# wenlinlee/FISCO-BCOS

Measured on AMD Instinct MI355X. Metric: sigs_per_sec, higher is better.
Workload: dtype u32 (256-bit integer); 1 GPU; C2; txs_total=10000, txs_rank0=10000, parallelism=dp1 (tx-index shards)

## Files before the change

fisco-bcos_amd/csrc/ecc_coop.hip:

```cpp
#include "ecc_device.h"
#include "ec26_trio.h"

namespace bcosgpu {

struct SplitLds {
    uint32_t tab[8][16][64];
    uint32_t zc[8][64];
    uint32_t u1[8][64];
    uint32_t k1[4][64];
    uint32_t k2[4][64];
    uint32_t flags[64];
    uint32_t pt[3][25][64];
};

__device__ __forceinline__ void lds_store_jac(uint32_t (*dst)[64], const Jac& P, int lane) {
    lds_store_fe(dst, P.X, lane);
    lds_store_fe(dst + 8, P.Y, lane);
    lds_store_fe(dst + 16, P.Z, lane);
    dst[24][lane] = P.inf ? 1u : 0u;
}
__device__ __forceinline__ void lds_load_jac(Jac& P, const uint32_t (*src)[64], int lane) {
    lds_load_fe(P.X, src, lane);
    lds_load_fe(P.Y, src + 8, lane);
    lds_load_fe(P.Z, src + 16, lane);
// ... 831 lines not shown
    for (int i = 0; i < lo; ++i) shr_bits<BITS>(k);
    CurveK1x::set_inf(acc);
    uint32_t b = k.v[0] & MASK;
    shr_bits<BITS>(k);
    const uint4* e = reinterpret_cast<const uint4*>(tab + (static_cast<size_t>(lo) * E + b) * 16);
    uint4 q0 = e[0], q1 = e[1], q2 = e[2], q3 = e[3];
#pragma unroll 1
    for (int i = lo; i < hi; ++i) {
        const uint32_t bi = b;
        Aff26 T;
        {
            const uint32_t x[8] = {q0.x, q0.y, q0.z, q0.w, q1.x, q1.y, q1.z, q1.w};
            const uint32_t y[8] = {q2.x, q2.y, q2.z, q2.w, q3.x, q3.y, q3.z, q3.w};
            fe26_from_words(T.x, x);
            fe26_from_words(T.y, y);
        }
        const int in = i + 1 < hi ? i + 1 : i;
        b = k.v[0] & MASK;
        shr_bits<BITS>(k);
        e = reinterpret_cast<const uint4*>(tab + (static_cast<size_t>(in) * E + b) * 16);
        q0 = e[0];
        q1 = e[1];
        q2 = e[2];
        q3 = e[3];
        Jac26 S;
        CurveK1x::madd(S, acc, T);
        CurveK1x::cmov(acc, S, bi != 0u);
    }
}

__device__ __forceinline__ void coop26_store_jac(uint32_t (*dst)[64], const Jac26& P, int lane) {
    fe X, Y, Z;
    fe26_to_fe(X, P.X);
    fe26_to_fe(Y, P.Y);
    fe26_to_fe(Z, P.Z);
    Jac J;
    fe_copy(J.X, X);
    fe_copy(J.Y, Y);
    fe_copy(J.Z, Z);
    J.inf = P.inf;
    coop_store_jac(dst, J, lane);
}
__device__ __forceinline__ void coop26_load_jac(Jac26& P, const uint32_t (*src)[64], int lane) {
    Jac J;
    coop_load_jac(J, src, lane);
    fe26_from_fe(P.X, J.X);
    fe26_from_fe(P.Y, J.Y);
    fe26_from_fe(P.Z, J.Z);
    P.inf = J.inf;
}
__device__ __forceinline__ void lds_load_fe26(fe26& a, const uint32_t (*src)[64], int lane) {
    fe w;
    lds_load_fe(w, src, lane);
    fe26_from_fe(a, w);
}
__device__ __forceinline__ void lds_store_fe26(uint32_t (*dst)[64], const fe26& a, int lane) {
    fe w;
    fe26_to_fe(w, a);
    lds_store_fe(dst, w, lane);
}

constexpr int kTrioWords = 31;
struct Trio26Lds {
    uint32_t tab[8][20][64];
    uint32_t tabphx[8][10][64];
    uint32_t zc[8][64];
    uint32_t k[2][4][64];
    uint32_t flags[64];
    uint32_t pt[5][25][64];
    uint32_t xe[8][64];
    uint32_t xrinv[8][64];
    uint32_t ys[8][64];
    uint32_t rflag[64];
    uint32_t post[3];
};
struct Trio26RecoverLds : Trio26Lds {
    uint32_t sq[10][40];
    uint32_t yok[64];
    uint32_t spost[kTfSlots];
    uint32_t hpost[4];
    uint32_t xg[2][kTrioWords][64];
    uint32_t tsuf[6][10][64];
    uint32_t kw[10][64];
};
__device__ __forceinline__ void lds_flag_wait4(uint32_t* a, uint32_t* b, uint32_t* c, uint32_t* d) {
    for (;;) {
        const uint32_t x = __hip_atomic_load(a, __ATOMIC_RELAXED, __HIP_MEMORY_SCOPE_WORKGROUP);
        const uint32_t y = __hip_atomic_load(b, __ATOMIC_RELAXED, __HIP_MEMORY_SCOPE_WORKGROUP);
        const uint32_t z = __hip_atomic_load(c, __ATOMIC_RELAXED, __HIP_MEMORY_SCOPE_WORKGROUP);
        const uint32_t u = __hip_atomic_load(d, __ATOMIC_RELAXED, __HIP_MEMORY_SCOPE_WORKGROUP);
        if (x != 0u && y != 0u && z != 0u && u != 0u) break;
        __builtin_amdgcn_s_sleep(1);
    }
    __builtin_amdgcn_fence(__ATOMIC_ACQUIRE, "workgroup");
}
struct TrioTableFlags {
    uint32_t* f;
    __device__ __forceinline__ void post(int s) { lds_flag_post(f + s); }
    __device__ __forceinline__ void wait(int s) { lds_flag_wait(f + s); }
    __device__ __forceinline__ void stamp(int k) {
        COOP_T(k);
        (void)k;
    }
};
__device__ __forceinline__ void lds_store_limbs26(uint32_t (*dst)[64], const fe26& a, int lane) {
    fe26 t;
    fe26_copy(t, a);
    fe26_normalize(t);
#pragma unroll
    for (int q = 0; q < 10; ++q) dst[q][lane] = t.v[q];
}

__device__ __forceinline__ void trio_store(uint32_t* buf, const TrioPt& P, int lane) {
#pragma unroll
    for (int q = 0; q < 10; ++q) {
        buf[q * 64 + lane] = P.S1.v[q];
        buf[(10 + q) * 64 + lane] = P.Xs.v[q];
        buf[(20 + q) * 64 + lane] = P.Zs.v[q];
    }
    buf[30 * 64 + lane] = P.inf ? 1u : 0u;
}
__device__ __forceinline__ void trio_load(TrioPt& P, const uint32_t* buf, int lane) {
#pragma unroll
    for (int q = 0; q < 10; ++q) {
        P.S1.v[q] = buf[q * 64 + lane];
        P.Xs.v[q] = buf[(10 + q) * 64 + lane];
        P.Zs.v[q] = buf[(20 + q) * 64 + lane];
    }
    P.inf = buf[30 * 64 + lane] != 0u;
}
__device__ __forceinline__ void trio_from_jac(TrioPt& P, const Jac26& J, const TrioLane& T) {
    trio::sel(P.S1, T.r0, J.X, J.Y);
    fe26_copy(P.Xs, J.X);
    fe26_copy(P.Zs, J.Z);
    P.inf = J.inf;
}

__device__ __forceinline__ void trio_entry(Aff26& S, const Trio26Lds& L, int tl, int d, bool neg, bool phi) {
    const uint32_t m = static_cast<uint32_t>((d < 0 ? -d : d) - 1) & 7u;
    const uint32_t* base = &L.tab[0][0][0] + m * (20 * 64) + tl;
    const uint32_t* bx = phi ? &L.tabphx[0][0][0] + m * (10 * 64) + tl : base;
#pragma unroll
    for (int q = 0; q < 10; ++q) {
        S.x.v[q] = bx[q * 64];
        S.y.v[q] = base[(10 + q) * 64];
    }
    F26_SETM(S.x, 1);
    F26_SETM(S.y, 1);
    fe26 ny;
    fe26_neg<2>(ny, S.y);
    fe26_cmov(S.y, ny, (d < 0) != neg);
}

__device__ __forceinline__ void trio_glv_chain(TrioPt& acc, const Trio26Lds& L, int chain, int tl, uint32_t tflags,
                                               const TrioLane& T) {
    fe k;
    fe_zero(k);
#pragma unroll
    for (int q = 0; q < 4; ++q) k.v[q] = L.k[chain][q][tl];
    const bool neg = chain == 0 ? (tflags & 4u) != 0 : (tflags & 8u) != 0;
    const bool phi = chain == 1;
    trio_chain_start(acc, k.v[3], [&](Aff26& S, int d) { trio_entry(S, L, tl, d, neg, phi); }, T);
    shl4_128(k);
    TrioAcc la;
    trio_acc_from(la, acc);
#pragma unroll 1
    for (int w = 30; w >= 0; --w)
        trio_window(la, booth_digit128(k), [&](Aff26& S, int d) { trio_entry(S, L, tl, d, neg, phi); }, T);
    trio_acc_to(acc, la, T);
}

template <bool WITH0, bool WITH2>
__device__ __forceinline__ void trio_sum_partials(TrioPt& A, const Trio26Lds& L, int tl, const TrioLane& T) {
    Jac26 Ga, Gb;
    TrioPt B;
    coop26_load_jac(Ga, L.pt[3], tl);
    coop26_load_jac(Gb, L.pt[4], tl);
    trio_from_jac(A, Ga, T);
    trio_from_jac(B, Gb, T);
    trio_add(A, A, B, T);
    if constexpr (WITH0) {
        coop26_load_jac(Gb, L.pt[0], tl);
        trio_from_jac(B, Gb, T);
        trio_add(A, A, B, T);
    }
    if constexpr (WITH2) {
        coop26_load_jac(Gb, L.pt[2], tl);
        trio_from_jac(B, Gb, T);
        trio_add(A, A, B, T);
    }
}


__device__ __forceinline__ bool recover_w(fe26& X, fe26& w, const fe& r, uint32_t v, bool ok) {
    fe x;
    fe_copy(x, r);
    bool okr = ok;
    if (v & 2u) {
        okr = okr && fe_lt_k(r, kK1PminusN);
        fe_add_k(x, r, ParamN1::M);
    }
    fe26 t, seven;
    fe26_from_fe(X, x);
    fe26_sqr(t, X);
    fe26_mul(w, t, X);
    fe26_set_small(seven, 7u);
    fe26_add(w, w, seven);
    return okr;
}

template <bool LIMBS, class LDS>
__device__ __forceinline__ void coop26_table_to_lds(LDS& L, const Aff26& P, int lane) {
    Aff26 A[8];
    fe26 Zc, beta;
    {
        Jac26 T[8];
        multiples8_26(T, P);
        coz_table26(A, Zc, T);
    }
    fe26_const(beta, kGlvBeta);
    Unroll<0, 8>::run([&](auto J) {
        constexpr int j = decltype(J)::value;
        fe26 bx;
        fe26_mul(bx, A[j].x, beta);
        if constexpr (LIMBS) {
            lds_store_limbs26(L.tab[j], A[j].x, lane);
            lds_store_limbs26(L.tab[j] + 10, A[j].y, lane);
            lds_store_limbs26(L.tabphx[j], bx, lane);
        } else {
            lds_store_fe26(L.tab[j], A[j].x, lane);
            lds_store_fe26(L.tab[j] + 8, A[j].y, lane);
            lds_store_fe26(L.tabphx[j], bx, lane);
        }
    });
    lds_store_fe26(L.zc, Zc, lane);
}

template <bool VERIFY, bool PIPE, class LDS, class IO>
__device__ __forceinline__ void coop26_post_e_inv(LDS& L, const IO& io, uint64_t i, bool active, bool ok, fe& r, fe& s,
                                                  int wave, int lane) {
    if (!ok) {
        fe_zero(r);
        r.v[0] = 1;
        fe_zero(s);
        if (VERIFY) s.v[0] = 1;
    }
    if (wave == 3) {
        fe e;
        fe_zero(e);
        if (active) io.template digest<KECCAK256>(i, e);
        reduce_once(e, ParamN1::M);
        lds_store_fe(L.xe, e, lane);
        lds_flag_post(&L.post[1]);
        COOP_T(7);
    } else if (wave == 0) {
        fe rm, rinv;
        FieldN1::from_plain(rm, VERIFY ? s : r);
        if constexpr (PIPE) FieldInv<FieldN1>::inv_pipe(rinv, rm);
        else FieldInv<FieldN1>::inv(rinv, rm);
        lds_store_fe(L.xrinv, rinv, lane);
        lds_flag_post(&L.post[0]);
        COOP_T(7);
    }
}
template <bool VERIFY, class LDS>
__device__ __forceinline__ void coop26_u1_glv(fe& u1, LDS& L, bool ok, const fe& r, const fe& s, int wave, int lane) {
    lds_flag_wait(&L.post[0]);
    lds_flag_wait(&L.post[1]);
    fe e, rinv;
    lds_load_fe(e, L.xe, lane);
    lds_load_fe(rinv, L.xrinv, lane);
    FieldN1::mul(u1, e, rinv);
    if (!VERIFY) FieldN1::neg(u1, u1);
    if (wave == 1) {
        fe u2, k1, k2;
        FieldN1::mul(u2, VERIFY ? r : s, rinv);
        bool neg1, neg2;
        glv_split(k1, neg1, k2, neg2, u2);
#pragma unroll
        for (int q = 0; q < 4; ++q) {
            L.k[0][q][lane] = k1.v[q];
            L.k[1][q][lane] = k2.v[q];
        }
        L.flags[lane] = (ok ? 1u : 0u) | (neg1 ? 4u : 0u) | (neg2 ? 8u : 0u);
    }
}

struct CombShare {
    int wide[4][2], narrow[4][2];
};
__device__ __forceinline__ void comb_share(int& lo, int& hi, const int (&t)[4][2], int wave) {
    lo = t[0][0];
    hi = t[0][1];
#pragma unroll
    for (int w = 1; w < 4; ++w) {
        if (wave == w) {
            lo = t[w][0];
            hi = t[w][1];
        }
    }
}
__device__ __forceinline__ void comb_share_range(Jac26& G, const fe& u1, const uint32_t* __restrict__ tab, int tab_bits,
                                                 const CombShare& share, int wave) {
    int lo, hi;
    if (tab_bits == kWideBits) {
        comb_share(lo, hi, share.wide, wave);
        comb_range26w<kWideBits>(G, u1, tab, lo, hi);
    } else {
        comb_share(lo, hi, share.narrow, wave);
        comb_range26w<8>(G, u1, tab, lo, hi);
    }
}
constexpr int kPairShare[4][2] = {{0, 12}, {24, 32}, {0, 0}, {12, 24}};
constexpr int kTrioSplitWin[3] = {5, 10, 16};
static_assert(0 < kTrioSplitWin[0] && kTrioSplitWin[0] < kTrioSplitWin[1] && kTrioSplitWin[1] < kTrioSplitWin[2] &&
                  kTrioSplitWin[2] <= 16,
              "comb windows of helpers 0, 1, 3, 2");
constexpr CombShare trio_recover_share() {
// ... 608 lines not shown
```

fisco-bcos_amd/csrc/ecc_device.h:

```cpp
#pragma once
#include <cstdlib>
#include <cstring>
#include <mutex>
#include <type_traits>
#include "ec.h"
#include "engine.h"
#include "hash_device.h"

namespace bcosgpu {

__device__ __constant__ static const uint32_t kK1Gx[8] = {0x16f81798u, 0x59f2815bu, 0x2dce28d9u, 0x029bfcdbu,
                                                       0xce870b07u, 0x55a06295u, 0xf9dcbbacu, 0x79be667eu};
__device__ __constant__ static const uint32_t kK1Gy[8] = {0xfb10d4b8u, 0x9c47d08fu, 0xa6855419u, 0xfd17b448u,
                                                       0x0e1108a8u, 0x5da4fbfcu, 0x26a3c465u, 0x483ada77u};
__device__ __constant__ static const uint32_t kK1PminusN[8] = {0x2fc9baeeu, 0x402da172u, 0x50b75fc4u, 0x45512319u,
                                                            0x00000001u, 0x00000000u, 0x00000000u, 0x00000000u};
__device__ __constant__ static const uint32_t kN1Half[8] = {0x681b20a0u, 0xdfe92f46u, 0x57a4501du, 0x5d576e73u,
                                                         0xffffffffu, 0xffffffffu, 0xffffffffu, 0x7fffffffu};
__device__ __constant__ static const uint32_t kGlvG1[8] = {0x45dbb031u, 0xe893209au, 0x71e8ca7fu, 0x3daa8a14u,
                                                        0x9284eb15u, 0xe86c90e4u, 0xa7d46bcdu, 0x3086d221u};
__device__ __constant__ static const uint32_t kGlvG2[8] = {0x8ac47f71u, 0x1571b4aeu, 0x9df506c6u, 0x221208acu,
                                                        0x0abfe4c4u, 0x6f547fa9u, 0x010e8828u, 0xe4437ed6u};
__device__ __constant__ static const uint32_t kGlvMB1[8] = {0x0abfe4c3u, 0x6f547fa9u, 0x010e8828u, 0xe4437ed6u,
                                                         0x00000000u, 0x00000000u, 0x00000000u, 0x00000000u};
__device__ __constant__ static const uint32_t kGlvMB2M[8] = {0x6a144696u, 0x0cac5e50u, 0xf3ba5939u, 0x1e8a8dc5u,
                                                          0xba244fceu, 0x176cdf65u, 0x8e173580u, 0xc25575ebu};
__device__ __constant__ static const uint32_t kGlvLambdaM[8] = {0xc9926c9eu, 0xf07deb3du, 0x83c6944cu, 0x2c93e7adu,
                                                             0x52697d91u, 0x73a96606u, 0x8558d639u, 0x53284017u};
__device__ __constant__ static const uint32_t kGlvBeta[8] = {0x719501eeu, 0xc1396c28u, 0x12f58995u, 0x9cf04975u,
                                                          0xac3434e9u, 0x6e64479eu, 0x657c0710u, 0x7ae96a2bu};
__device__ __constant__ static const uint32_t kSM2Gx[8] = {0xf418029eu, 0x61328990u, 0xdca6c050u, 0x3e7981edu,
                                                        0xac24c3c3u, 0xd6a1ed99u, 0xe1c13b05u, 0x91167a5eu};
__device__ __constant__ static const uint32_t kSM2Gy[8] = {0x3c2d0dddu, 0xc1354e59u, 0x8d3295fau, 0xc1f5e578u,
                                                        0x6e2a48f8u, 0x8d4cfb06u, 0x81d735bdu, 0x63cd65d4u};
__device__ __constant__ static const uint32_t kSM2B[8] = {0x2bc0dd42u, 0x90d23063u, 0xe9b537abu, 0x71cf379au,
                                                       0x5ea51c3cu, 0x52798150u, 0xba20e2c8u, 0x240fe188u};
__device__ __constant__ static const uint32_t kZaMid[8] = {0xadadedb5u, 0x0446043fu, 0x08a87aceu, 0xe86d2243u,
                                                        0x8e232383u, 0xbfc81fe2u, 0xcf9117c8u, 0x4707011du};
__device__ __constant__ static const uint32_t kZaW32[4] = {0x2153d0a9u, 0x877cc62au, 0x474002dfu, 0x32e52139u};
static constexpr uint32_t kZaC36 = 0xf0a00000u;

static constexpr int kCombWindows = 32;
static constexpr int kCombEntries = 256;
static constexpr size_t kTabWords = static_cast<size_t>(kCombWindows) * kCombEntries * 16;
static constexpr int kWideBits = 16;
static constexpr int kWideWindows = 256 / kWideBits;
static constexpr uint32_t kWideEntries = 1u << kWideBits;
static constexpr size_t kWideTabWords = static_cast<size_t>(kWideWindows) * kWideEntries * 16;

__device__ __forceinline__ void load_be256(fe& r, const uint8_t* p) {
    ByteReader rd(p, 32);
    uint32_t w[8];
#pragma unroll
    for (int i = 0; i < 8; ++i) w[i] = rd.word(i);
    fe_from_be_words(r, w);
}
__device__ __forceinline__ void load_be256_aligned(fe& r, const uint8_t* p) {
    const uint4* q = reinterpret_cast<const uint4*>(p);
    const uint4 a = q[0], b = q[1];
    const uint32_t w[8] = {a.x, a.y, a.z, a.w, b.x, b.y, b.z, b.w};
    fe_from_be_words(r, w);
}
__device__ __forceinline__ void store_be256(uint8_t* p, const fe& a) {
    uint32_t w[8];
    fe_to_be_words(w, a);
    uint4* q = reinterpret_cast<uint4*>(p);
    q[0] = make_uint4(w[0], w[1], w[2], w[3]);
    q[1] = make_uint4(w[4], w[5], w[6], w[7]);
}
__device__ __forceinline__ void store_be256_u32(uint8_t* p, const fe& a) {
    uint32_t w[8];
    fe_to_be_words(w, a);
    uint32_t* q = reinterpret_cast<uint32_t*>(p);
#pragma unroll
    for (int i = 0; i < 8; ++i) q[i] = w[i];
}
__device__ __forceinline__ void shr8(fe& k) {
#pragma unroll
    for (int i = 0; i < 7; ++i) k.v[i] = __builtin_amdgcn_alignbit(k.v[i + 1], k.v[i], 8);
    k.v[7] >>= 8;
}
__device__ __forceinline__ void shl4(fe& k) {
#pragma unroll
    for (int i = 7; i > 0; --i) k.v[i] = __builtin_amdgcn_alignbit(k.v[i], k.v[i - 1], 28);
    k.v[0] <<= 4;
}
__device__ __forceinline__ void shl1(fe& k) {
#pragma unroll
    for (int i = 7; i > 0; --i) k.v[i] = __builtin_amdgcn_alignbit(k.v[i], k.v[i - 1], 31);
    k.v[0] <<= 1;
}
__device__ __forceinline__ void shl4_128(fe& k) {
#pragma unroll
    for (int i = 3; i > 0; --i) k.v[i] = __builtin_amdgcn_alignbit(k.v[i], k.v[i - 1], 28);
    k.v[0] <<= 4;
}
__device__ __forceinline__ int booth_digit256(fe& k) {
    const uint32_t top = k.v[7];
    const uint32_t W = top >> 28, c = (top >> 27) & 1u;
    shl4(k);
    return static_cast<int>(W + c) - static_cast<int>((W >> 3) << 4);
}
__device__ __forceinline__ int booth_digit128(fe& k) {
    const uint32_t top = k.v[3];
    const uint32_t W = top >> 28, c = (top >> 27) & 1u;
    shl4_128(k);
    return static_cast<int>(W + c) - static_cast<int>((W >> 3) << 4);
}
__device__ __forceinline__ void reduce_once(fe& x, const uint32_t* n) {
    fe t;
    const uint32_t bw = fe_sub_k(t, x, n);
    fe_cmov(x, t, bw == 0);
}

template <int BITS>
__device__ __forceinline__ void shr_bits(fe& k) {
#pragma unroll
    for (int i = 0; i < 7; ++i) k.v[i] = __builtin_amdgcn_alignbit(k.v[i + 1], k.v[i], BITS);
    k.v[7] >>= BITS;
}
__device__ __forceinline__ void load_aff16(Aff& T, const uint32_t* __restrict__ e32) {
    const uint4* e = reinterpret_cast<const uint4*>(e32);
    const uint4 q0 = e[0], q1 = e[1], q2 = e[2], q3 = e[3];
    T.x.v[0] = q0.x; T.x.v[1] = q0.y; T.x.v[2] = q0.z; T.x.v[3] = q0.w;
    T.x.v[4] = q1.x; T.x.v[5] = q1.y; T.x.v[6] = q1.z; T.x.v[7] = q1.w;
    T.y.v[0] = q2.x; T.y.v[1] = q2.y; T.y.v[2] = q2.z; T.y.v[3] = q2.w;
    T.y.v[4] = q3.x; T.y.v[5] = q3.y; T.y.v[6] = q3.z; T.y.v[7] = q3.w;
}

template <class C, int BITS = kWideBits>
__device__ __forceinline__ void comb_mul(Jac& acc, const fe& k_plain, const uint32_t* __restrict__ tab) {
    constexpr int W = 256 / BITS;
    constexpr uint32_t E = 1u << BITS, MASK = E - 1u;
    fe k;
    fe_copy(k, k_plain);
    C::set_inf(acc);
    uint32_t b = k.v[0] & MASK;
    shr_bits<BITS>(k);
    Aff T;
    load_aff16(T, tab + static_cast<size_t>(b) * 16);
#pragma unroll 1
    for (int i = 0; i < W; ++i) {
        const uint32_t bi = b;
        Aff N;
        const int in = i + 1 < W ? i + 1 : i;
        b = k.v[0] & MASK;
        shr_bits<BITS>(k);
        load_aff16(N, tab + (static_cast<size_t>(in) * E + b) * 16);
        Jac S;
        C::madd(S, acc, T);
        C::cmov(acc, S, bi != 0u);
        fe_copy(T.x, N.x);
        fe_copy(T.y, N.y);
    }
}

struct CombTab {
    const uint32_t* p;
    int bits;
};

template <class C>
__device__ __forceinline__ void comb_mul_rt(Jac& acc, const fe& k, const uint32_t* __restrict__ tab, int tbits) {
    if (tbits == kWideBits) comb_mul<C, kWideBits>(acc, k, tab);
    else comb_mul<C, 8>(acc, k, tab);
}

template <class C, class F>
__device__ __forceinline__ void booth_mul(Jac& acc, const fe& k_plain, const Aff& P) {
    Jac T[8];
    C::from_aff(T[0], P);
    C::dbl(T[1], T[0]);
    C::madd(T[2], T[1], P);
    C::dbl(T[3], T[1]);
    C::madd(T[4], T[3], P);
    C::dbl(T[5], T[2]);
    C::madd(T[6], T[5], P);
    C::dbl(T[7], T[3]);
    fe k;
    fe_copy(k, k_plain);
    C::set_inf(acc);
    C::cmov(acc, T[0], (k.v[7] >> 31) != 0u);
#pragma unroll 1
    for (int i = 63; i >= 0; --i) {
        C::dbl(acc, acc);
        C::dbl(acc, acc);
        C::dbl(acc, acc);
        C::dbl(acc, acc);
        const int d = booth_digit256(k);
        const uint32_t m = static_cast<uint32_t>((d < 0 ? -d : d) - 1) & 7u;
        Jac S;
        fe_copy(S.X, T[0].X); fe_copy(S.Y, T[0].Y); fe_copy(S.Z, T[0].Z); S.inf = false;
#pragma unroll
        for (int q = 1; q < 8; ++q) {
            const bool take = m == static_cast<uint32_t>(q);
            fe_cmov(S.X, T[q].X, take);
            fe_cmov(S.Y, T[q].Y, take);
            fe_cmov(S.Z, T[q].Z, take);
        }
        fe ny;
        F::neg(ny, S.Y);
        fe_cmov(S.Y, ny, d < 0);
        Jac R;
        C::add(R, acc, S);
        C::cmov(acc, R, d != 0);
    }
}

__device__ __forceinline__ void glv_split(fe& k1, bool& neg1, fe& k2, bool& neg2, const fe& k) {
    uint32_t t[16];
    fe g, c1, c2, x, y;
    fe_set(g, kGlvG1);
    mul_512(t, k, g);
    uint32_t c = 0;
#pragma unroll
    for (int i = 0; i < 4; ++i) c1.v[i] = addc32(t[12 + i], i == 0 ? (t[11] >> 31) : 0u, c, c);
#pragma unroll
    for (int i = 4; i < 8; ++i) c1.v[i] = 0;
    fe_set(g, kGlvG2);
    mul_512(t, k, g);
    c = 0;
#pragma unroll
    for (int i = 0; i < 4; ++i) c2.v[i] = addc32(t[12 + i], i == 0 ? (t[11] >> 31) : 0u, c, c);
#pragma unroll
    for (int i = 4; i < 8; ++i) c2.v[i] = 0;
    fe_set(g, kGlvMB1);
    mul_512(t, c1, g);
#pragma unroll
    for (int i = 0; i < 8; ++i) x.v[i] = t[i];
    reduce_once(x, ParamN1::M);
    fe_set(g, kGlvMB2M);
    FieldN1::mul(y, c2, g);
    FieldN1::add(k2, x, y);
    fe_set(g, kGlvLambdaM);
    FieldN1::mul(x, k2, g);
    FieldN1::sub(k1, k, x);
    fe half, nk;
    fe_set(half, kN1Half);
    neg1 = fe_lt(half, k1);
    FieldN1::neg(nk, k1);
    fe_cmov(k1, nk, neg1);
    neg2 = fe_lt(half, k2);
    FieldN1::neg(nk, k2);
    fe_cmov(k2, nk, neg2);
}

template <class C, class F>
__device__ __forceinline__ void add_digit_aff(Jac& acc, const Aff T[8], int d, bool neg, bool phi) {
    const uint32_t m = static_cast<uint32_t>((d < 0 ? -d : d) - 1) & 7u;
    Aff S;
    fe_copy(S.x, T[0].x);
    fe_copy(S.y, T[0].y);
#pragma unroll
    for (int q = 1; q < 8; ++q) {
        const uint64_t take = __builtin_amdgcn_ballot_w64(m == static_cast<uint32_t>(q));
        fe_cmov_mask(S.x, T[q].x, take);
        fe_cmov_mask(S.y, T[q].y, take);
    }
    if (phi) {
        fe b;
        fe_set(b, kGlvBeta);
        F::mul(S.x, S.x, b);
    }
    fe ny;
    F::neg(ny, S.y);
    fe_cmov(S.y, ny, (d < 0) != neg);
    Jac R;
    C::madd(R, acc, S);
    C::cmov(acc, R, d != 0);
}

template <class C, class F>
__device__ __forceinline__ void add_digit_ldsx(Jac& acc, const uint32_t* ldsx, const fe Y[8], int d, bool neg,
                                               bool phi) {
    const uint32_t m = static_cast<uint32_t>((d < 0 ? -d : d) - 1) & 7u;
    Aff S;
    const uint32_t* b = ldsx + m * 512u;
#pragma unroll
    for (int k = 0; k < 8; ++k) S.x.v[k] = b[k * 64];
    fe_copy(S.y, Y[0]);
#pragma unroll
    for (int q = 1; q < 8; ++q) fe_cmov_mask(S.y, Y[q], __builtin_amdgcn_ballot_w64(m == static_cast<uint32_t>(q)));
    if (phi) {
        fe bt;
        fe_set(bt, kGlvBeta);
        F::mul(S.x, S.x, bt);
    }
    fe ny;
    F::neg(ny, S.y);
    fe_cmov(S.y, ny, (d < 0) != neg);
    Jac R;
    C::madd(R, acc, S);
    C::cmov(acc, R, d != 0);
}

__device__ __forceinline__ void table_x_to_lds(uint32_t* ldsx, const Aff A[8], fe Y[8]) {
#pragma unroll
    for (int j = 0; j < 8; ++j) {
#pragma unroll
        for (int k = 0; k < 8; ++k) ldsx[(j * 8 + k) * 64] = A[j].x.v[k];
        fe_copy(Y[j], A[j].y);
    }
}

template <class C>
__device__ __forceinline__ void multiples8(Jac T[8], const Aff& P) {
    C::from_aff(T[0], P);
    C::dbl(T[1], T[0]);
    C::madd(T[2], T[1], P);
    C::dbl(T[3], T[1]);
    C::madd(T[4], T[3], P);
    C::dbl(T[5], T[2]);
    C::madd(T[6], T[5], P);
    C::dbl(T[7], T[3]);
}

template <int I, int N>
struct Unroll {
    template <class Fn>
    __device__ static __forceinline__ void run(Fn&& fn) {
        if constexpr (I < N) {
            fn(std::integral_constant<int, I>{});
            Unroll<I + 1, N>::run(fn);
        }
    }
};

__device__ __forceinline__ void coz_table_k1(Aff A[8], fe& Zc, const Jac T[8]) {
    fe pre[8], suf[8];
    FieldK1::set_one(pre[0]);
    fe_copy(pre[1], T[1].Z);
    Unroll<2, 8>::run([&](auto J) { FieldK1::mul(pre[J], pre[J - 1], T[J].Z); });
    FieldK1::set_one(suf[7]);
    Unroll<0, 7>::run([&](auto J) {
        constexpr int j = 6 - decltype(J)::value;
        FieldK1::mul(suf[j], suf[j + 1], T[j + 1].Z);
    });
    fe_copy(Zc, pre[7]);
    Unroll<0, 8>::run([&](auto J) {
        constexpr int j = decltype(J)::value;
        fe sj, s2, s3;
        if constexpr (j == 0) fe_copy(sj, suf[0]);
        else if constexpr (j == 7) fe_copy(sj, pre[6]);
        else FieldK1::mul(sj, pre[j - 1], suf[j]);
        FieldK1::sqr(s2, sj);
        FieldK1::mul(s3, s2, sj);
        FieldK1::mul(A[j].x, T[j].X, s2);
        FieldK1::mul(A[j].y, T[j].Y, s3);
    });
}

template <bool LDS = false>
__device__ __forceinline__ void glv_mul_k1(Jac& acc, const fe& k, const Aff& P, uint32_t* ldsx = nullptr) {
    fe k1, k2, Zc;
    bool neg1, neg2;
    glv_split(k1, neg1, k2, neg2, k);
    Aff A[8];
    {
        Jac T[8];
        multiples8<CurveK1>(T, P);
        coz_table_k1(A, Zc, T);
    }
    CurveK1::set_inf(acc);
    if constexpr (LDS) {
        fe Y[8];
        table_x_to_lds(ldsx, A, Y);
        add_digit_ldsx<CurveK1, FieldK1>(acc, ldsx, Y, static_cast<int>(k1.v[3] >> 31), neg1, false);
        add_digit_ldsx<CurveK1, FieldK1>(acc, ldsx, Y, static_cast<int>(k2.v[3] >> 31), neg2, true);
#pragma unroll 1
        for (int i = 31; i >= 0; --i) {
            CurveK1::dbl(acc, acc);
            CurveK1::dbl(acc, acc);
            CurveK1::dbl(acc, acc);
            CurveK1::dbl(acc, acc);
            const int d1 = booth_digit128(k1);
            const int d2 = booth_digit128(k2);
            add_digit_ldsx<CurveK1, FieldK1>(acc, ldsx, Y, d1, neg1, false);
            add_digit_ldsx<CurveK1, FieldK1>(acc, ldsx, Y, d2, neg2, true);
        }
        FieldK1::mul(acc.Z, acc.Z, Zc);
        return;
    }
    add_digit_aff<CurveK1, FieldK1>(acc, A, static_cast<int>(k1.v[3] >> 31), neg1, false);
    add_digit_aff<CurveK1, FieldK1>(acc, A, static_cast<int>(k2.v[3] >> 31), neg2, true);
#pragma unroll 1
    for (int i = 31; i >= 0; --i) {
        CurveK1::dbl(acc, acc);
        CurveK1::dbl(acc, acc);
        CurveK1::dbl(acc, acc);
        CurveK1::dbl(acc, acc);
        const int d1 = booth_digit128(k1);
        const int d2 = booth_digit128(k2);
        add_digit_aff<CurveK1, FieldK1>(acc, A, d1, neg1, false);
        add_digit_aff<CurveK1, FieldK1>(acc, A, d2, neg2, true);
    }
    FieldK1::mul(acc.Z, acc.Z, Zc);
}
// ... 672 lines not shown
```

fisco-bcos_amd/csrc/modinv.h:

```cpp
#pragma once
#include "fe.h"
#include "modinv30.h"

namespace bcosgpu {

__device__ __constant__ static const ModInfo30 kMod30K1P = {
    {1073740847, 1073741819, 1073741823, 1073741823, 1073741823, 1073741823, 1073741823, 1073741823, 65535}, 769313487u};
__device__ __constant__ static const ModInfo30 kMod30N1 = {
    {271991105, 1061780019, 881460155, 733428139, 1073741498, 1073741823, 1073741823, 1073741823, 65535}, 712462017u};
__device__ __constant__ static const ModInfo30 kMod30P2 = {
    {1073741823, 1073741823, 15, 1073741760, 1073741823, 1073741823, 1073741823, 1073725439, 65535}, 1073741823u};
__device__ __constant__ static const ModInfo30 kMod30N2 = {
    {970277155, 250597412, 476074677, 16243400, 1073741682, 1073741823, 1073741823, 1073725439, 65535}, 231405195u};

__device__ __forceinline__ void fe_to_s30(S30& r, const fe& a) {
#pragma unroll
    for (int i = 0; i < 8; ++i) {
        const int bit = 30 * i, w = bit >> 5, sh = bit & 31;
        uint32_t x = a.v[w] >> sh;
        if (sh > 2 && w + 1 < 8) x |= a.v[w + 1] << (32 - sh);
        r.v[i] = static_cast<int32_t>(x & kM30);
    }
    r.v[8] = static_cast<int32_t>(a.v[7] >> 16);
}
// ... 141 lines not shown
    update_fg_30(f, g, t);
#pragma unroll 1
    for (int it = 1; it < 25; ++it) {
        int32_t gz = 0;
#pragma unroll
        for (int i = 0; i < 9; ++i) gz |= g.v[i];
        if (__builtin_amdgcn_ballot_w64(gz != 0) == 0) break;
        int32_t tp[4] = {t[0], t[1], t[2], t[3]};
        eta = divsteps_30_var<U>(eta, static_cast<uint32_t>(f.v[0]), static_cast<uint32_t>(g.v[0]), t);
        update_de_30(d, e, tp, mi);
        update_fg_30(f, g, t);
    }
    update_de_30(d, e, t, mi);
    normalize_30(d, f.v[8], mi);
    s30_to_fe(r, d);
}

struct InvQueue {
    int32_t t[25][4];
    int32_t d[9];
    uint32_t n, done, ready;
};
__device__ __forceinline__ void invq_reset(InvQueue& q) {
    q.n = 0u;
    q.done = 0u;
    q.ready = 0u;
}
__device__ __forceinline__ int32_t modinv_var_split_fg(const fe& x, const ModInfo30& mi, InvQueue& q, int lane) {
    S30 f, g;
#pragma unroll
    for (int i = 0; i < 9; ++i) f.v[i] = mi.m[i];
    fe_to_s30(g, x);
    int32_t eta = -1;
#pragma unroll 1
    for (int it = 0; it < 25; ++it) {
        int32_t t[4];
        eta = divsteps_30_var(eta, static_cast<uint32_t>(f.v[0]), static_cast<uint32_t>(g.v[0]), t);
        if (lane == 0) {
#pragma unroll
            for (int k = 0; k < 4; ++k) q.t[it][k] = t[k];
            __hip_atomic_store(&q.n, static_cast<uint32_t>(it + 1), __ATOMIC_RELEASE, __HIP_MEMORY_SCOPE_WORKGROUP);
        }
        update_fg_30(f, g, t);
        int32_t gz = 0;
#pragma unroll
        for (int i = 0; i < 9; ++i) gz |= g.v[i];
        if (__builtin_amdgcn_ballot_w64(gz != 0) == 0) break;
    }
    if (lane == 0) __hip_atomic_store(&q.done, 1u, __ATOMIC_RELEASE, __HIP_MEMORY_SCOPE_WORKGROUP);
    return f.v[8];
}
__device__ __forceinline__ void modinv_var_split_de(const ModInfo30& mi, InvQueue& q, int lane) {
    S30 d, e;
#pragma unroll
    for (int i = 0; i < 9; ++i) {
        d.v[i] = 0;
        e.v[i] = 0;
    }
    e.v[0] = 1;
#pragma unroll 1
    for (uint32_t b = 0; b < 25u; ++b) {
        uint32_t n;
        for (;;) {
            n = __builtin_amdgcn_readfirstlane(__hip_atomic_load(&q.n, __ATOMIC_ACQUIRE, __HIP_MEMORY_SCOPE_WORKGROUP));
            if (n > b) break;
            if (__builtin_amdgcn_readfirstlane(
                    __hip_atomic_load(&q.done, __ATOMIC_ACQUIRE, __HIP_MEMORY_SCOPE_WORKGROUP)) != 0u) {
                n = __builtin_amdgcn_readfirstlane(__hip_atomic_load(&q.n, __ATOMIC_ACQUIRE, __HIP_MEMORY_SCOPE_WORKGROUP));
                break;
            }
            __builtin_amdgcn_s_sleep(1);
        }
        if (n <= b) break;
        int32_t t[4];
#pragma unroll
        for (int k = 0; k < 4; ++k) t[k] = q.t[b][k];
        update_de_30(d, e, t, mi);
    }
    if (lane == 0) {
#pragma unroll
        for (int i = 0; i < 9; ++i) q.d[i] = d.v[i];
        __hip_atomic_store(&q.ready, 1u, __ATOMIC_RELEASE, __HIP_MEMORY_SCOPE_WORKGROUP);
    }
}
__device__ __forceinline__ void modinv_var_split_finish(fe& r, int32_t fsign, const ModInfo30& mi, InvQueue& q) {
    while (__hip_atomic_load(&q.ready, __ATOMIC_ACQUIRE, __HIP_MEMORY_SCOPE_WORKGROUP) == 0u)
        __builtin_amdgcn_s_sleep(1);
    S30 d;
#pragma unroll
    for (int i = 0; i < 9; ++i) d.v[i] = q.d[i];
    normalize_30(d, fsign, mi);
    s30_to_fe(r, d);
}

__device__ __constant__ static const uint32_t kR3P2[8] = {0x00000016u, 0x00000012u, 0xfffffff8u, 0x0000000eu,
                                                       0x0000000cu, 0x0000000au, 0x00000009u, 0x0000001bu};
__device__ __constant__ static const uint32_t kR3N1[8] = {0xe9ff41edu, 0x7bc0cfe0u, 0x44d4322cu, 0x00176484u,
                                                       0xf1d0b2dau, 0xb1b31347u, 0x18ef116du, 0x555d800cu};
__device__ __constant__ static const uint32_t kR3N2[8] = {0x0eaa0b85u, 0x6ff874c7u, 0xaabe8d32u, 0x87d0c315u,
                                                       0x97185afcu, 0x4c4fbbb3u, 0xd574ea14u, 0xc813249cu};

template <class F>
struct FieldInv;
template <>
struct FieldInv<FieldK1> {
    __device__ static __forceinline__ void inv(fe& r, const fe& a) {
        fe t;
        fe_copy(t, a);
        FieldK1::normalize(t);
        modinv_safegcd(r, t, kMod30K1P);
    }
    __device__ static __forceinline__ void inv_pipe(fe& r, const fe& a) {
        fe t;
        fe_copy(t, a);
        FieldK1::normalize(t);
        modinv_safegcd_pipe(r, t, kMod30K1P);
    }
    __device__ static __forceinline__ void inv_var(fe& r, const fe& a) {
        fe t;
        fe_copy(t, a);
        FieldK1::normalize(t);
        modinv_safegcd_var(r, t, kMod30K1P);
    }
    template <int SRC, int DST>
    __device__ static __forceinline__ void inv_trio(fe& r, const fe& a, const TrioLane& T, int lane) {
        fe t;
        fe_copy(t, a);
        FieldK1::normalize(t);
        modinv_trio<SRC, DST>(r, t, kMod30K1P, T, lane);
    }
};
template <class P, int PIPE = 0>
__device__ __forceinline__ void mont_inv_safegcd(fe& r, const fe& a, const ModInfo30& mi, const uint32_t* r3) {
    fe t, k;
    if constexpr (PIPE == 2) modinv_safegcd_var(t, a, mi);
    else if constexpr (PIPE == 1) modinv_safegcd_pipe(t, a, mi);
    else modinv_safegcd(t, a, mi);
    fe_set(k, r3);
    Mont<P>::mul(r, t, k);
}
template <>
struct FieldInv<FieldP2> {
    __device__ static __forceinline__ void inv(fe& r, const fe& a) { mont_inv_safegcd<ParamP2>(r, a, kMod30P2, kR3P2); }
};
template <>
struct FieldInv<FieldN1> {
    __device__ static __forceinline__ void inv(fe& r, const fe& a) { mont_inv_safegcd<ParamN1>(r, a, kMod30N1, kR3N1); }
    __device__ static __forceinline__ void inv_pipe(fe& r, const fe& a) {
        mont_inv_safegcd<ParamN1, 1>(r, a, kMod30N1, kR3N1);
    }
    __device__ static __forceinline__ void inv_var(fe& r, const fe& a) {
        mont_inv_safegcd<ParamN1, 2>(r, a, kMod30N1, kR3N1);
    }
};
template <>
struct FieldInv<FieldN2> {
    __device__ static __forceinline__ void inv(fe& r, const fe& a) { mont_inv_safegcd<ParamN2>(r, a, kMod30N2, kR3N2); }
};

}
```

Baseline: 31.67 million tx/s (hash + recover/verify + sender).

## Compute GLV split with 160-bit integer arithmetic and align trio window loop

Replaces the modular GLV scalar split (full 512-bit products, Montgomery multiplies mod n, negation and compare) with a plain-integer version. It multiplies only the needed low 160 bits and takes sign and magnitude straight from two's-complement differences. The trio GLV chain loop head is also padded with s_nops and aligned to a 64-byte boundary to control instruction-fetch alignment. A new inv_trio helper for cooperative n1 inversion is added but has no caller here. The risk is correctness at edge cases of the integer split, and a loop alignment that may not hold after other code changes.

```diff
diff --git a/fisco-bcos_amd/csrc/ecc_coop.hip b/fisco-bcos_amd/csrc/ecc_coop.hip
--- a/fisco-bcos_amd/csrc/ecc_coop.hip
+++ b/fisco-bcos_amd/csrc/ecc_coop.hip
@@ -1007,6 +1007,10 @@
     fe26_cmov(S.y, ny, (d < 0) != neg);
 }
 
+static constexpr int kTrioLoopPad = 2;
+static constexpr int kTrioLoopHeadMod64 = 12;
+static_assert(kTrioLoopHeadMod64 == (4 * kTrioLoopPad + 4) % 64, "the pad, then one preheader instruction");
+
 __device__ __forceinline__ void trio_glv_chain(TrioPt& acc, const Trio26Lds& L, int chain, int tl, uint32_t tflags,
                                                const TrioLane& T) {
     fe k;
@@ -1019,6 +1023,7 @@
     shl4_128(k);
     TrioAcc la;
     trio_acc_from(la, acc);
+    asm volatile(".p2align 6\n\t.rept %0\n\ts_nop 0\n\t.endr" ::"n"(kTrioLoopPad));
 #pragma unroll 1
     for (int w = 30; w >= 0; --w)
         trio_window(la, booth_digit128(k), [&](Aff26& S, int d) { trio_entry(S, L, tl, d, neg, phi); }, T);
diff --git a/fisco-bcos_amd/csrc/ecc_device.h b/fisco-bcos_amd/csrc/ecc_device.h
--- a/fisco-bcos_amd/csrc/ecc_device.h
+++ b/fisco-bcos_amd/csrc/ecc_device.h
@@ -5,6 +5,7 @@
 #include <type_traits>
 #include "ec.h"
 #include "engine.h"
+#include "glv_split.h"
 #include "hash_device.h"
 
 namespace bcosgpu {
@@ -17,16 +18,6 @@
                                                             0x00000001u, 0x00000000u, 0x00000000u, 0x00000000u};
 __device__ __constant__ static const uint32_t kN1Half[8] = {0x681b20a0u, 0xdfe92f46u, 0x57a4501du, 0x5d576e73u,
                                                          0xffffffffu, 0xffffffffu, 0xffffffffu, 0x7fffffffu};
-__device__ __constant__ static const uint32_t kGlvG1[8] = {0x45dbb031u, 0xe893209au, 0x71e8ca7fu, 0x3daa8a14u,
-                                                        0x9284eb15u, 0xe86c90e4u, 0xa7d46bcdu, 0x3086d221u};
-__device__ __constant__ static const uint32_t kGlvG2[8] = {0x8ac47f71u, 0x1571b4aeu, 0x9df506c6u, 0x221208acu,
-                                                        0x0abfe4c4u, 0x6f547fa9u, 0x010e8828u, 0xe4437ed6u};
-__device__ __constant__ static const uint32_t kGlvMB1[8] = {0x0abfe4c3u, 0x6f547fa9u, 0x010e8828u, 0xe4437ed6u,
-                                                         0x00000000u, 0x00000000u, 0x00000000u, 0x00000000u};
-__device__ __constant__ static const uint32_t kGlvMB2M[8] = {0x6a144696u, 0x0cac5e50u, 0xf3ba5939u, 0x1e8a8dc5u,
-                                                          0xba244fceu, 0x176cdf65u, 0x8e173580u, 0xc25575ebu};
-__device__ __constant__ static const uint32_t kGlvLambdaM[8] = {0xc9926c9eu, 0xf07deb3du, 0x83c6944cu, 0x2c93e7adu,
-                                                             0x52697d91u, 0x73a96606u, 0x8558d639u, 0x53284017u};
 __device__ __constant__ static const uint32_t kGlvBeta[8] = {0x719501eeu, 0xc1396c28u, 0x12f58995u, 0x9cf04975u,
                                                           0xac3434e9u, 0x6e64479eu, 0x657c0710u, 0x7ae96a2bu};
 __device__ __constant__ static const uint32_t kSM2Gx[8] = {0xf418029eu, 0x61328990u, 0xdca6c050u, 0x3e7981edu,
@@ -208,41 +199,12 @@
 }
 
 __device__ __forceinline__ void glv_split(fe& k1, bool& neg1, fe& k2, bool& neg2, const fe& k) {
-    uint32_t t[16];
-    fe g, c1, c2, x, y;
-    fe_set(g, kGlvG1);
-    mul_512(t, k, g);
-    uint32_t c = 0;
-#pragma unroll
-    for (int i = 0; i < 4; ++i) c1.v[i] = addc32(t[12 + i], i == 0 ? (t[11] >> 31) : 0u, c, c);
-#pragma unroll
-    for (int i = 4; i < 8; ++i) c1.v[i] = 0;
-    fe_set(g, kGlvG2);
-    mul_512(t, k, g);
-    c = 0;
-#pragma unroll
-    for (int i = 0; i < 4; ++i) c2.v[i] = addc32(t[12 + i], i == 0 ? (t[11] >> 31) : 0u, c, c);
-#pragma unroll
-    for (int i = 4; i < 8; ++i) c2.v[i] = 0;
-    fe_set(g, kGlvMB1);
-    mul_512(t, c1, g);
-#pragma unroll
-    for (int i = 0; i < 8; ++i) x.v[i] = t[i];
-    reduce_once(x, ParamN1::M);
-    fe_set(g, kGlvMB2M);
-    FieldN1::mul(y, c2, g);
-    FieldN1::add(k2, x, y);
-    fe_set(g, kGlvLambdaM);
-    FieldN1::mul(x, k2, g);
-    FieldN1::sub(k1, k, x);
-    fe half, nk;
-    fe_set(half, kN1Half);
-    neg1 = fe_lt(half, k1);
-    FieldN1::neg(nk, k1);
-    fe_cmov(k1, nk, neg1);
-    neg2 = fe_lt(half, k2);
-    FieldN1::neg(nk, k2);
-    fe_cmov(k2, nk, neg2);
+    uint32_t n1, n2;
+    glv_split_core(k1.v, n1, k2.v, n2, k.v);
+#pragma unroll
+    for (int i = 4; i < 8; ++i) k1.v[i] = k2.v[i] = 0;
+    neg1 = n1 != 0u;
+    neg2 = n2 != 0u;
 }
 
 template <class C, class F>
diff --git a/fisco-bcos_amd/csrc/glv_split.h b/fisco-bcos_amd/csrc/glv_split.h
--- /dev/null
+++ b/fisco-bcos_amd/csrc/glv_split.h
@@ -0,0 +1,104 @@
+#pragma once
+#include "fe26.h"
+
+#if defined(__HIPCC__) || defined(__HIP__)
+#define GLV_TABLE __device__ __constant__ static const uint32_t
+#else
+#define GLV_TABLE static const uint32_t
+#endif
+
+namespace bcosgpu {
+
+GLV_TABLE kGlvG1[8] = {0x45dbb031u, 0xe893209au, 0x71e8ca7fu, 0x3daa8a14u,
+                       0x9284eb15u, 0xe86c90e4u, 0xa7d46bcdu, 0x3086d221u};
+GLV_TABLE kGlvG2[8] = {0x8ac47f71u, 0x1571b4aeu, 0x9df506c6u, 0x221208acu,
+                       0x0abfe4c4u, 0x6f547fa9u, 0x010e8828u, 0xe4437ed6u};
+GLV_TABLE kGlvMB1[4] = {0x0abfe4c3u, 0x6f547fa9u, 0x010e8828u, 0xe4437ed6u};
+GLV_TABLE kGlvA1[4] = {0x9284eb15u, 0xe86c90e4u, 0xa7d46bcdu, 0x3086d221u};
+GLV_TABLE kGlvA2[5] = {0x9d44cfd8u, 0x57c1108du, 0xa8e2f3f6u, 0x14ca50f7u, 0x00000001u};
+
+F26_HD void glv_round_mul(uint32_t c[4], const uint32_t k[8], const uint32_t* g) {
+    uint32_t t[16];
+#pragma unroll
+    for (int i = 0; i < 16; ++i) t[i] = 0;
+#pragma unroll
+    for (int i = 0; i < 8; ++i) {
+        uint32_t carry = 0;
+#pragma unroll
+        for (int j = 0; j < 8; ++j) {
+            const uint64_t p = static_cast<uint64_t>(k[i]) * g[j] + t[i + j] + carry;
+            t[i + j] = static_cast<uint32_t>(p);
+            carry = static_cast<uint32_t>(p >> 32);
+        }
+        t[i + 8] = carry;
+    }
+    uint64_t s = static_cast<uint64_t>(t[11] >> 31);
+#pragma unroll
+    for (int i = 0; i < 4; ++i) {
+        s += t[12 + i];
+        c[i] = static_cast<uint32_t>(s);
+        s >>= 32;
+    }
+}
+
+template <int NB>
+F26_HD void glv_mul_lo160(uint32_t r[5], const uint32_t c[4], const uint32_t* m) {
+#pragma unroll
+    for (int i = 0; i < 5; ++i) r[i] = 0;
+#pragma unroll
+    for (int i = 0; i < 4; ++i) {
+        uint32_t carry = 0;
+#pragma unroll
+        for (int j = 0; j < NB; ++j) {
+            if (i + j < 4) {
+                const uint64_t p = static_cast<uint64_t>(c[i]) * m[j] + r[i + j] + carry;
+                r[i + j] = static_cast<uint32_t>(p);
+                carry = static_cast<uint32_t>(p >> 32);
+            } else if (i + j == 4) {
+                r[4] += c[i] * m[j] + carry;
+                carry = 0;
+            }
+        }
+        if (i + NB <= 4) r[i + NB] = carry;
+    }
+}
+
+F26_HD void glv_sub160(uint32_t r[5], const uint32_t a[5], const uint32_t b[5]) {
+    uint32_t bw = 0;
+#pragma unroll
+    for (int i = 0; i < 5; ++i) {
+        const uint64_t d = static_cast<uint64_t>(a[i]) - b[i] - bw;
+        r[i] = static_cast<uint32_t>(d);
+        bw = static_cast<uint32_t>(d >> 32) & 1u;
+    }
+}
+
+F26_HD void glv_sign_mag(uint32_t mag[4], uint32_t& neg, const uint32_t x[5]) {
+    neg = x[4] >> 31;
+    const uint32_t m = 0u - neg;
+    uint64_t s = neg;
+#pragma unroll
+    for (int i = 0; i < 4; ++i) {
+        s += x[i] ^ m;
+        mag[i] = static_cast<uint32_t>(s);
+        s >>= 32;
+    }
+}
+
+F26_HD void glv_split_core(uint32_t k1[4], uint32_t& neg1, uint32_t k2[4], uint32_t& neg2, const uint32_t k[8]) {
+    uint32_t c1[4], c2[4];
+    glv_round_mul(c1, k, kGlvG1);
+    glv_round_mul(c2, k, kGlvG2);
+    uint32_t p[5], q[5], x[5];
+    glv_mul_lo160<4>(p, c1, kGlvMB1);
+    glv_mul_lo160<4>(q, c2, kGlvA1);
+    glv_sub160(x, p, q);
+    glv_sign_mag(k2, neg2, x);
+    glv_mul_lo160<4>(p, c1, kGlvA1);
+    glv_mul_lo160<5>(q, c2, kGlvA2);
+    glv_sub160(x, k, p);
+    glv_sub160(x, x, q);
+    glv_sign_mag(k1, neg1, x);
+}
+
+}
diff --git a/fisco-bcos_amd/csrc/modinv.h b/fisco-bcos_amd/csrc/modinv.h
--- a/fisco-bcos_amd/csrc/modinv.h
+++ b/fisco-bcos_amd/csrc/modinv.h
@@ -317,6 +317,13 @@
     __device__ static __forceinline__ void inv_var(fe& r, const fe& a) {
         mont_inv_safegcd<ParamN1, 2>(r, a, kMod30N1, kR3N1);
     }
+    template <int SRC, int DST>
+    __device__ static __forceinline__ void inv_trio(fe& r, const fe& a, const TrioLane& T, int lane) {
+        fe t, k;
+        modinv_trio<SRC, DST>(t, a, kMod30N1, T, lane);
+        fe_set(k, kR3N1);
+        Mont<ParamN1>::mul(r, t, k);
+    }
 };
 template <>
 struct FieldInv<FieldN2> {
```

Result: faster. 32.49 million tx/s (hash + recover/verify + sender), median of 6 (+2.6%).
